# RatInABox-Lab/RatInABox

Measured on AMD Instinct MI355X. Metric: agent-steps/sec (whole node) at 4096 agents x 1024 PlaceCells, higher is better.
Workload: dtype f32 rates / f64 motion

## Files before the change

ratinabox_amd/csrc/riab_handover.h:

```cpp
#pragma once
#include "riab_device.h"

namespace riab {

typedef __attribute__((address_space(1))) uint32_t riab_g32;
typedef __attribute__((address_space(1))) unsigned long long riab_g64;

__device__ __forceinline__ void st_agent(uint32_t* p, uint32_t v) {
  __hip_atomic_store((riab_g32*)(uintptr_t)p, v, __ATOMIC_RELAXED, __HIP_MEMORY_SCOPE_AGENT);
}
__device__ __forceinline__ uint32_t ld_agent(const uint32_t* p) {
  return __hip_atomic_load((riab_g32*)(uintptr_t)p, __ATOMIC_RELAXED, __HIP_MEMORY_SCOPE_AGENT);
}
__device__ __forceinline__ void st_agent(int32_t* p, int32_t v) { st_agent(reinterpret_cast<uint32_t*>(p), (uint32_t)v); }
__device__ __forceinline__ int32_t ld_agent(const int32_t* p) { return (int32_t)ld_agent(reinterpret_cast<const uint32_t*>(p)); }
__device__ __forceinline__ void st_agent(uint64_t* p, uint64_t v) {
  __hip_atomic_store((riab_g64*)(uintptr_t)p, (unsigned long long)v, __ATOMIC_RELAXED, __HIP_MEMORY_SCOPE_AGENT);
}
__device__ __forceinline__ uint64_t ld_agent(const uint64_t* p) {
  return (uint64_t)__hip_atomic_load((riab_g64*)(uintptr_t)p, __ATOMIC_RELAXED, __HIP_MEMORY_SCOPE_AGENT);
}
__device__ __forceinline__ void st_agent(double* p, double v) { st_agent(reinterpret_cast<uint64_t*>(p), (uint64_t)__double_as_longlong(v)); }
__device__ __forceinline__ double ld_agent(const double* p) {
  return __longlong_as_double((long long)ld_agent(reinterpret_cast<const uint64_t*>(p)));
}
__device__ __forceinline__ void st_agent(float* p, float v) { st_agent(reinterpret_cast<uint32_t*>(p), __float_as_uint(v)); }
__device__ __forceinline__ void st_agent(uint8_t* p, uint8_t v) {
  __hip_atomic_store((__attribute__((address_space(1))) uint8_t*)(uintptr_t)p, v, __ATOMIC_RELAXED, __HIP_MEMORY_SCOPE_AGENT);
}
__device__ __forceinline__ uint32_t fetch_add_agent(uint32_t* p, uint32_t v) {
  return __hip_atomic_fetch_add((riab_g32*)(uintptr_t)p, v, __ATOMIC_RELAXED, __HIP_MEMORY_SCOPE_AGENT);
}
__device__ __forceinline__ int32_t fetch_add_agent(int32_t* p, int32_t v) {
  return (int32_t)fetch_add_agent(reinterpret_cast<uint32_t*>(p), (uint32_t)v);
}
__device__ __forceinline__ uint64_t fetch_max_agent(uint64_t* p, uint64_t v) {
  return (uint64_t)__hip_atomic_fetch_max((riab_g64*)(uintptr_t)p, (unsigned long long)v, __ATOMIC_RELAXED, __HIP_MEMORY_SCOPE_AGENT);
}

__device__ __forceinline__ void st_agent_v4f(void* p, riab_v4f v) {
  riab_g64* const g = (riab_g64*)(uintptr_t)p;
  __hip_atomic_store(g, ((unsigned long long)__float_as_uint(v.y) << 32) | __float_as_uint(v.x), __ATOMIC_RELAXED, __HIP_MEMORY_SCOPE_AGENT);
  __hip_atomic_store(g + 1, ((unsigned long long)__float_as_uint(v.w) << 32) | __float_as_uint(v.z), __ATOMIC_RELAXED, __HIP_MEMORY_SCOPE_AGENT);
}
__device__ __forceinline__ riab_v4f ld_agent_v4f(const void* p) {
  riab_g64* const g = (riab_g64*)(uintptr_t)p;
  const unsigned long long lo = __hip_atomic_load(g, __ATOMIC_RELAXED, __HIP_MEMORY_SCOPE_AGENT);
  const unsigned long long hi = __hip_atomic_load(g + 1, __ATOMIC_RELAXED, __HIP_MEMORY_SCOPE_AGENT);
  return riab_v4f{__uint_as_float((uint32_t)lo), __uint_as_float((uint32_t)(lo >> 32)), __uint_as_float((uint32_t)hi),
                  __uint_as_float((uint32_t)(hi >> 32))};
}

__device__ __forceinline__ void drain_stores() { asm volatile("s_waitcnt vmcnt(0)" ::: "memory"); }
#define RIAB_WAITCNT_VMCNT0 0x0F70
__device__ __forceinline__ void drain_stores_nofence_asm() {
  __atomic_signal_fence(__ATOMIC_SEQ_CST);
  __builtin_amdgcn_s_waitcnt(RIAB_WAITCNT_VMCNT0);
  __atomic_signal_fence(__ATOMIC_SEQ_CST);
}

__device__ __forceinline__ uint64_t mail_word(uint32_t epoch, uint32_t v) { return ((uint64_t)epoch << 32) | v; }
__device__ __forceinline__ bool mail_fresh(uint64_t e, uint32_t epoch) { return (uint32_t)(e >> 32) == epoch; }

}
```

ratinabox_amd/csrc/riab_rate_cells.h:

```cpp
#pragma once
#include "riab_device.h"
#include "riab_handover.h"

namespace riab {

typedef float v4f __attribute__((ext_vector_type(4)));
typedef float v2f __attribute__((ext_vector_type(2)));

struct SpikeCtx {
  uint8_t* spikes;
  const float* u_in;
  float dt;
  uint32_t k0, k1;
  uint32_t tag;
};

struct RateArgs {
  const float* pos_x;
  const float* pos_y;
  const float* hd_x;
  const float* hd_y;
  int64_t pos_ld;
  int64_t nquads;
  int64_t qrow;
  int64_t B;
  float* rates;
  uint8_t* spikes;
  const float* u_in;
  float dt, fr_scale, fr_min;
  uint32_t k0, k1;
  uint32_t step0;
  uint32_t tag;
  uint32_t group0;
  int32_t n;
  int32_t cells_per_block;
  __device__ __forceinline__ SpikeCtx spike_ctx() const { return SpikeCtx{spikes, u_in, dt, k0, k1, tag}; }
};

struct PosQuad {
  v4f x, y;
};

__device__ __forceinline__ v4f ldv4(const float* p) { return *reinterpret_cast<const v4f*>(p); }

__device__ __forceinline__ v4f finish_rate(v4f r, const PosQuad& P) {
  r.x = (P.x.x == P.x.x) ? r.x : 0.0f;
  r.y = (P.x.y == P.x.y) ? r.y : 0.0f;
  r.z = (P.x.z == P.x.z) ? r.z : 0.0f;
  r.w = (P.x.w == P.x.w) ? r.w : 0.0f;
  return r;
}
template <class P_>
__device__ __forceinline__ v4f finish_rate(v4f r, const P_&) { return r; }

template <class Cell>
__device__ __forceinline__ v4f post_scale(const Cell&, const float*, const typename Cell::Pos&, v4f r) { return r; }

template <bool EXPLICIT_U, int POLICY = RIAB_STORE_NT>
__device__ __forceinline__ void spike_store(const SpikeCtx& a, v4f r, int64_t off, uint32_t step, uint32_t c,
                                            uint32_t group) {
  v4f u;
  if (EXPLICIT_U) {
    u = ldv4(a.u_in + off);
  } else {
    const u32x4 w = philox4x32_spikes(step, c, group, a.tag, a.k0, a.k1);
    u = v4f{u01_24(w.x), u01_24(w.y), u01_24(w.z), u01_24(w.w)};
  }
  const uint32_t s = (u.x < a.dt * r.x ? 1u : 0u) | (u.y < a.dt * r.y ? 0x100u : 0u) |
                     (u.z < a.dt * r.z ? 0x10000u : 0u) | (u.w < a.dt * r.w ? 0x1000000u : 0u);
  store_stream<POLICY>(reinterpret_cast<uint32_t*>(a.spikes + off), s);
}

template <int DESC, int GX>
struct PlaceCell {
  typedef PosQuad Pos;
  static constexpr int LDS_DOUBLES = (GX == 1 || GX == 2) ? 4 * RIAB_MAX_WALLS + 8 : 1;
  const float* tab;
  float scale, half_scale;
  float top_hat_w2;
  const double* walls;
  int n_internal;
  double e0, e1, e2, e3;
  EnvShape shape;
  const double* lds;

  __device__ __forceinline__ void stage(double* s) {
    lds = s;
    if (GX == 1 || GX == 2) {
      for (int i = threadIdx.x; i < 4 * n_internal; i += 256) s[i] = walls[16 + i];
      __syncthreads();
    }
  }
  __device__ __forceinline__ Pos load(const RateArgs& a, int64_t off) const {
    return Pos{ldv4(a.pos_x + off), ldv4(a.pos_y + off)};
  }
  __device__ __forceinline__ Pos load_agent(const RateArgs& a, int64_t off) const {
    return Pos{ld_agent_v4f(a.pos_x + off), ld_agent_v4f(a.pos_y + off)};
  }
  __device__ __forceinline__ Pos from_rows(v4f x, v4f y, v4f, v4f) const { return Pos{x, y}; }
  static constexpr bool NEEDS_HD = false;
  static constexpr bool NEEDS_POS = true;
  __device__ __forceinline__ float wrap(float v) const {
    const float av = fabsf(v);
    return (av > half_scale) ? -copysignf(scale - av, v) : v;
  }
  __device__ __forceinline__ float dist2(float cxs, float cys, float px, float py) const {
    float dx = cxs - px, dy = cys - py;
    if (GX == 3) {
      dx = wrap(dx);
      dy = wrap(dy);
    }
    float d2 = fmaf(dy, dy, dx * dx);
    if (GX == 1) {
      bool blocked = false;
      for (int w = 0; w < n_internal; ++w)
        blocked |= seg_hit(cxs, cys, px, py, lds[4 * w], lds[4 * w + 1], lds[4 * w + 2], lds[4 * w + 3]);
      if (blocked) d2 = 1.0e6f;
    }
    if (GX == 2) {
      if (n_internal > 0 && seg_hit(cxs, cys, px, py, lds[0], lds[1], lds[2], lds[3])) {
        float best = INFINITY;
        bool any = false;
#pragma unroll
        for (int e = 0; e < 2; ++e) {
          const double exd = lds[2 * e], eyd = lds[2 * e + 1];
          if (env_contains(shape, exd, eyd, [&](int k, double& ax, double& ay, double& bx, double& by) {
                ax = walls[4 * k]; ay = walls[4 * k + 1]; bx = walls[4 * k + 2]; by = walls[4 * k + 3];
              })) {
            const float ex = (float)exd, ey = (float)eyd;
            const float d1 = sqrtf(fmaf(cys - ey, cys - ey, (cxs - ex) * (cxs - ex)));
            const float d2e = sqrtf(fmaf(ey - py, ey - py, (ex - px) * (ex - px)));
            best = fminf(best, d1 + d2e);
            any = true;
          }
        }
        if (any) d2 = best * best;
      }
    }
    return d2;
  }
  __device__ __forceinline__ float fr(float d2, float ks) const {
    if (DESC == RIAB_PC_GAUSSIAN) return __builtin_amdgcn_exp2f(d2 * ks);
    if (DESC == RIAB_PC_GAUSSIAN_THRESHOLD) {
      const float e12 = 0.60653065971263342f;
      return fmaxf(__builtin_amdgcn_exp2f(d2 * ks) - e12, 0.0f) * (1.0f / (1.0f - e12));
    }
    if (DESC == RIAB_PC_DIFF_OF_GAUSSIANS) {
      const float g1 = __builtin_amdgcn_exp2f(d2 * ks);
      const float g2 = __builtin_amdgcn_exp2f(d2 * ks * (1.0f / 2.25f));
      return (g1 - (1.0f / 2.25f) * g2) * (2.25f / 1.25f);
    }
    if (DESC == RIAB_PC_TOP_HAT) return (d2 < top_hat_w2) ? 1.0f : 0.0f;
    return 0.0f;
  }
  static constexpr int NP = 3;
  static constexpr int CPB = 4;
  __device__ __forceinline__ v4f eval(const float* p, const Pos& P) const {
    const float cxs = p[0], cys = p[1], ks = p[2];
    v4f r;
    r.x = fr(dist2(cxs, cys, P.x.x, P.y.x), ks);
    r.y = fr(dist2(cxs, cys, P.x.y, P.y.y), ks);
    r.z = fr(dist2(cxs, cys, P.x.z, P.y.z), ks);
    r.w = fr(dist2(cxs, cys, P.x.w, P.y.w), ks);
    return r;
  }
  template <int D2>
  __host__ PlaceCell<D2, GX> as() const;
};
template <int DESC, int GX>
__host__ __device__ __forceinline__ PlaceCell<DESC, GX> place_cell(const float* tab, float scale, float half_scale, float top_hat_w2,
                                                                   const double* walls = nullptr, int n_internal = 0,
                                                                   const EnvShape& shape = EnvShape{}) {
  PlaceCell<DESC, GX> c;
  c.tab = tab; c.scale = scale; c.half_scale = half_scale; c.top_hat_w2 = top_hat_w2;
  c.walls = walls; c.n_internal = n_internal;
  c.e0 = shape.e0; c.e1 = shape.e1; c.e2 = shape.e2; c.e3 = shape.e3; c.shape = shape; c.lds = nullptr;
  return c;
}
template <int DESC, int GX>
template <int D2>
__host__ PlaceCell<D2, GX> PlaceCell<DESC, GX>::as() const {
  return place_cell<D2, GX>(tab, scale, half_scale, top_hat_w2, walls, n_internal, shape);
}

struct ThetaPos {
  PosQuad q;
  v4f dx, dy;
};

template <int DESC, int GX>
struct ThetaPlaceCell {
  typedef ThetaPos Pos;
  static constexpr int LDS_DOUBLES = 1;
  __device__ __forceinline__ void stage(double*) {}
  PlaceCell<DESC, GX> base;
  const float* tab;
  const double* vx64;
  const double* vy64;
  float phase0;
  float k2;
  float norm;
  __device__ __forceinline__ Pos load(const RateArgs& a, int64_t off) const {
    Pos P;
    P.q = base.load(a, off);
    const double* px = vx64 + off;
    const double* py = vy64 + off;
    const v4f vx = {(float)px[0], (float)px[1], (float)px[2], (float)px[3]};
    const v4f vy = {(float)py[0], (float)py[1], (float)py[2], (float)py[3]};
    const v4f sp{sqrtf(fmaf(vy.x, vy.x, vx.x * vx.x)), sqrtf(fmaf(vy.y, vy.y, vx.y * vx.y)),
                 sqrtf(fmaf(vy.z, vy.z, vx.z * vx.z)), sqrtf(fmaf(vy.w, vy.w, vx.w * vx.w))};
    const v4f inv = 1.0f / (sp + 1e-8f);
    P.dx = vx * inv;
    P.dy = vy * inv;
    return P;
  }
  static constexpr int NP = 4;
  static constexpr int CPB = 4;
  __device__ __forceinline__ v4f eval(const float* p, const Pos& P) const { return base.eval(p, P.q); }
  __device__ __forceinline__ float factor(float cx, float cy, float pf, float px, float py, float dx, float dy) const {
    const float along = fmaf(py - cy, dy, (px - cx) * dx);
    float rev = fmaf(-along, pf, phase0);
    rev -= floorf(rev);
    return __builtin_amdgcn_exp2f((__builtin_amdgcn_cosf(rev) - 1.0f) * k2) * norm;
  }
  __device__ __forceinline__ v4f modulation(const float* p, const Pos& P) const {
    return v4f{factor(p[0], p[1], p[3], P.q.x.x, P.q.y.x, P.dx.x, P.dy.x), factor(p[0], p[1], p[3], P.q.x.y, P.q.y.y, P.dx.y, P.dy.y),
               factor(p[0], p[1], p[3], P.q.x.z, P.q.y.z, P.dx.z, P.dy.z), factor(p[0], p[1], p[3], P.q.x.w, P.q.y.w, P.dx.w, P.dy.w)};
  }
};

template <int DESC, int GX>
__device__ __forceinline__ v4f post_scale(const ThetaPlaceCell<DESC, GX>& c, const float* p, const ThetaPos& P, v4f r) {
  return r * c.modulation(p, P);
}
__device__ __forceinline__ v4f finish_rate(v4f r, const ThetaPos& P) { return finish_rate(r, P.q); }

template <int DESC>
struct GridCell {
  typedef PosQuad Pos;
  static constexpr int LDS_DOUBLES = 1;
  __device__ __forceinline__ void stage(double*) {}
  const float* tab;
  float f0, inv_1mf0;
  __device__ __forceinline__ Pos load(const RateArgs& a, int64_t off) const {
    return Pos{ldv4(a.pos_x + off), ldv4(a.pos_y + off)};
  }
  __device__ __forceinline__ Pos load_agent(const RateArgs& a, int64_t off) const {
    return Pos{ld_agent_v4f(a.pos_x + off), ld_agent_v4f(a.pos_y + off)};
  }
  __device__ __forceinline__ Pos from_rows(v4f x, v4f y, v4f, v4f) const { return Pos{x, y}; }
  static constexpr bool NEEDS_HD = false;
  static constexpr bool NEEDS_POS = true;
  __device__ __forceinline__ v2f two(const float* p, v2f x, v2f y) const {
    v2f s = {0.0f, 0.0f};
#pragma unroll
    for (int i = 0; i < 3; ++i) {
      const v2f p0 = {p[3 * i], p[3 * i]}, p1 = {p[3 * i + 1], p[3 * i + 1]}, p2 = {p[3 * i + 2], p[3 * i + 2]};
      v2f rev = p0 - __builtin_elementwise_fma(x, p1, y * p2);
      rev.x -= floorf(rev.x);
      rev.y -= floorf(rev.y);
      s += v2f{__builtin_amdgcn_cosf(rev.x), __builtin_amdgcn_cosf(rev.y)};
    }
    s *= v2f{1.0f / 3.0f, 1.0f / 3.0f};
    if (DESC == RIAB_GC_RECTIFIED) {
      const v2f r = (s - v2f{f0, f0}) * v2f{inv_1mf0, inv_1mf0};
      return v2f{fmaxf(r.x, 0.0f), fmaxf(r.y, 0.0f)};
    }
    return v2f{2.0f / 3.0f, 2.0f / 3.0f} * (s + v2f{0.5f, 0.5f});
  }
  static constexpr int NP = 9;
  static constexpr int CPB = 4;
  __device__ __forceinline__ v4f eval(const float* p, const Pos& P) const {
    const v2f lo = two(p, v2f{P.x.x, P.x.y}, v2f{P.y.x, P.y.y});
    const v2f hi = two(p, v2f{P.x.z, P.x.w}, v2f{P.y.z, P.y.w});
    return v4f{lo.x, lo.y, hi.x, hi.y};
  }
};

struct PlaneWaveCell {
  typedef PosQuad Pos;
  static constexpr int LDS_DOUBLES = 1;
  __device__ __forceinline__ void stage(double*) {}
  const float* tab;
  __device__ __forceinline__ Pos load(const RateArgs& a, int64_t off) const {
    return Pos{ldv4(a.pos_x + off), ldv4(a.pos_y + off)};
  }
  __device__ __forceinline__ Pos load_agent(const RateArgs& a, int64_t off) const {
    return Pos{ld_agent_v4f(a.pos_x + off), ld_agent_v4f(a.pos_y + off)};
  }
  __device__ __forceinline__ Pos from_rows(v4f x, v4f y, v4f, v4f) const { return Pos{x, y}; }
  static constexpr bool NEEDS_HD = false;
  static constexpr bool NEEDS_POS = true;
  __device__ __forceinline__ v2f two(const float* p, v2f x, v2f y) const {
#pragma clang fp contract(off)
    const v2f p0 = {p[0], p[0]}, p1 = {p[1], p[1]}, p2 = {p[2], p[2]};
    v2f rev = p0 - __builtin_elementwise_fma(x, p1, y * p2);
    rev.x -= floorf(rev.x);
    rev.y -= floorf(rev.y);
    const v2f c = {__builtin_amdgcn_cosf(rev.x), __builtin_amdgcn_cosf(rev.y)};
    return __builtin_elementwise_fma(v2f{0.5f, 0.5f}, c, v2f{0.5f, 0.5f});
  }
  static constexpr int NP = 3;
  static constexpr int CPB = 4;
  __device__ __forceinline__ v4f eval(const float* p, const Pos& P) const {
    const v2f lo = two(p, v2f{P.x.x, P.x.y}, v2f{P.y.x, P.y.y});
    const v2f hi = two(p, v2f{P.x.z, P.x.w}, v2f{P.y.z, P.y.w});
    return v4f{lo.x, lo.y, hi.x, hi.y};
  }
};

template <int MODE>
struct HDCell {
  struct Pos {
    v4f cs, sn;
    v4f speed;
  };
  static constexpr int LDS_DOUBLES = 1;
  __device__ __forceinline__ void stage(double*) {}
  const float* tab;
  float speed_inv;
  const double* vx64;
  const double* vy64;
  __device__ __forceinline__ Pos load_agent(const RateArgs& a, int64_t off) const {
    return from_dirs(ld_agent_v4f(a.hd_x + off), ld_agent_v4f(a.hd_y + off));
  }
  __device__ __forceinline__ Pos from_rows(v4f, v4f, v4f hx, v4f hy) const { return from_dirs(hx, hy); }
  static constexpr bool NEEDS_HD = true;
  static constexpr bool NEEDS_POS = false;
  __device__ __forceinline__ Pos load(const RateArgs& a, int64_t off) const {
    v4f hx, hy;
    if (MODE == 1 && vx64) {
      const double* px = vx64 + off;
      const double* py = vy64 + off;
      hx = v4f{(float)px[0], (float)px[1], (float)px[2], (float)px[3]};
      hy = v4f{(float)py[0], (float)py[1], (float)py[2], (float)py[3]};
    } else {
      hx = ldv4(a.hd_x + off);
      hy = ldv4(a.hd_y + off);
    }
    return from_dirs(hx, hy);
  }
  __device__ __forceinline__ Pos from_dirs(v4f hx, v4f hy) const {
    Pos P;
    if (MODE >= 1) {
      const v4f sp{sqrtf(fmaf(hy.x, hy.x, hx.x * hx.x)), sqrtf(fmaf(hy.y, hy.y, hx.y * hx.y)),
                   sqrtf(fmaf(hy.z, hy.z, hx.z * hx.z)), sqrtf(fmaf(hy.w, hy.w, hx.w * hx.w))};
      P.speed = sp * speed_inv;
      if (MODE == 1) {
        hx = hx / sp;
        hy = hy / sp;
      }
    } else {
      P.speed = v4f{1.0f, 1.0f, 1.0f, 1.0f};
    }
    {
#pragma clang fp contract(off)
      const v4f bx = hx + 1e-6f;
      const v4f inv = {1.0f / sqrtf(fmaf(hy.x, hy.x, bx.x * bx.x)), 1.0f / sqrtf(fmaf(hy.y, hy.y, bx.y * bx.y)),
                       1.0f / sqrtf(fmaf(hy.z, hy.z, bx.z * bx.z)), 1.0f / sqrtf(fmaf(hy.w, hy.w, bx.w * bx.w))};
      P.cs = bx * inv;
      P.sn = hy * inv;
    }
    return P;
  }
  static constexpr int NP = 3;
  static constexpr int CPB = 16;
  __device__ __forceinline__ v4f eval(const float* p, const Pos& P) const {
#pragma clang fp contract(off)
    if (MODE == 2) return P.speed;
    const float cp = p[0], sp = p[1], k2 = p[2];
    const v4f cosd = __builtin_elementwise_fma(P.cs, v4f{cp, cp, cp, cp}, P.sn * sp);
    const v4f dc = P.cs - cp, ds = P.sn - sp;
    const v4f chord = __builtin_elementwise_fma(ds, ds, dc * dc) * -0.5f;
    const v4f prod = cosd - 1.0f;
    const v4f e = v4f{cosd.x > 0.75f ? chord.x : prod.x, cosd.y > 0.75f ? chord.y : prod.y, cosd.z > 0.75f ? chord.z : prod.z,
                      cosd.w > 0.75f ? chord.w : prod.w} * k2;
    return v4f{__builtin_amdgcn_exp2f(e.x), __builtin_amdgcn_exp2f(e.y), __builtin_amdgcn_exp2f(e.z),
               __builtin_amdgcn_exp2f(e.w)};
  }
};

__device__ __forceinline__ v4f finish_rate(v4f r, const HDCell<1>::Pos& P) { return r * P.speed; }

#define RIAB_CELL_GROUP(Cell, CPB, cell, mine, P, c0, n, fr_scale, fr_min, rates, off, ld, store, RATE_POLICY, PHILOX,       \
                        EXPLICIT, SPIKE_POLICY, ctx, step, group)                                                         \
  {                                                                                                                        \
    static_assert(Cell::NP * (CPB) <= 64, "a cell group's parameters must fit one wave");                                  \
    _Pragma("unroll") for (int j_ = 0; j_ < (CPB); ++j_) {                                                                 \
      if ((c0) + j_ < (n)) {                                                                             \
        float p_[Cell::NP];                                                                                                \
        _Pragma("unroll") for (int i_ = 0; i_ < Cell::NP; ++i_) p_[i_] = __builtin_bit_cast(                               \
            float, __builtin_amdgcn_readlane(__builtin_bit_cast(int, mine), j_ * Cell::NP + i_));                          \
        v4f r_ = (cell).eval(p_, P);                                                                                       \
        r_ = finish_rate(post_scale(cell, p_, P, r_ * (fr_scale) + (fr_min)), P);           \
        if (store) {                                                                                                       \
          store_stream<(RATE_POLICY)>((rates) + (off), r_);                                                                \
          if (PHILOX) spike_store<false, (SPIKE_POLICY)>(ctx, r_, off, step, (uint32_t)((c0) + j_), group);                \
          if (EXPLICIT) spike_store<true, (SPIKE_POLICY)>(ctx, r_, off, step, (uint32_t)((c0) + j_), group);               \
        }                                                                                                                  \
        (off) += (ld);                                                                                                     \
      }                                                                                                                    \
    }                                                                                                                      \
  }

}
```

ratinabox_amd/csrc/riab_rates.hip:

```cpp
#include <hip/hip_ext.h>

#include <type_traits>

#include "riab_device.h"
#include "riab_rate_cells.h"
#include "riab_handover.h"
#include "riab_launch.h"
#ifndef RIAB_SPIKE_POLICY_GATED
#define RIAB_SPIKE_POLICY_GATED RIAB_STORE_NT
#endif
#ifndef RIAB_SPIKE_POLICY_WIDE
#define RIAB_SPIKE_POLICY_WIDE RIAB_STORE_NT
#endif

namespace riab {


template <class Cell, int SPK, int CPB, bool NT>
__global__ __launch_bounds__(256) void rate_kernel_wide(const RateArgs a, Cell cell) {
  __shared__ double s_lds[Cell::LDS_DOUBLES];
  cell.stage(s_lds);
  constexpr int NP = Cell::NP;
  const int lane = threadIdx.x & 63;
  const int c0 = blockIdx.y * CPB;
  const uint32_t t = blockIdx.z;
  const uint32_t q = blockIdx.x * 256u + threadIdx.x;
  const bool live = q < (uint32_t)a.qrow;
  const uint32_t qc = live ? q : 0u;
  const int pi = c0 * NP + lane;
  const float mine = (lane < NP * CPB && pi < a.n * NP) ? cell.tab[pi] : 0.0f;
  const typename Cell::Pos P = cell.load(a, (int64_t)t * a.pos_ld + 4 * (int64_t)qc);
  int64_t off = ((int64_t)t * a.n + c0) * a.B + 4 * (int64_t)qc;
  const uint32_t step = a.step0 + t;
  const uint32_t group = a.group0 + qc;
  const SpikeCtx k = a.spike_ctx();
  RIAB_CELL_GROUP(Cell, CPB, cell, mine, P, c0, a.n, a.fr_scale, a.fr_min, a.rates, off, a.B, live,
                  NT ? RIAB_STORE_WT : RIAB_STORE_PLAIN, SPK == 1, SPK == 2, NT ? RIAB_STORE_WT : RIAB_SPIKE_POLICY_WIDE, k, step, group)
}

template <class Cell, int SPK>
__global__ __launch_bounds__(256) void rate_kernel_generic(const RateArgs a, Cell cell) {
  __shared__ double s_lds[Cell::LDS_DOUBLES];
  cell.stage(s_lds);
  constexpr int NP = Cell::NP;
  const uint32_t p4 = blockIdx.x * 256u + threadIdx.x;
  const bool live = p4 < a.nquads;
  const uint32_t pc = live ? p4 : 0u;
  const uint32_t t = pc / (uint32_t)a.qrow;
  const uint32_t q = pc - t * (uint32_t)a.qrow;
  const typename Cell::Pos P = cell.load(a, (int64_t)t * a.pos_ld + 4 * (int64_t)q);
  const int c0 = blockIdx.y * a.cells_per_block;
  const int c1 = min(a.n, c0 + a.cells_per_block);
  int64_t off = ((int64_t)t * a.n + c0) * a.B + 4 * (int64_t)q;
  const uint32_t step = a.step0 + t;
  const uint32_t group = a.group0 + q;
  const int lane = threadIdx.x & 63;
  for (int cb = c0; cb < c1; cb += 64) {
    float mine[NP];
    const int cm = min(cb + lane, a.n - 1);
#pragma unroll
    for (int i = 0; i < NP; ++i) mine[i] = cell.tab[cm * NP + i];
    const int cnt = min(64, c1 - cb);
    for (int j = 0; j < cnt; ++j) {
      float p[NP];
#pragma unroll
      for (int i = 0; i < NP; ++i)
        p[i] = __builtin_bit_cast(float, __builtin_amdgcn_readlane(__builtin_bit_cast(int, mine[i]), j));
      v4f r = cell.eval(p, P);
      r = finish_rate(post_scale(cell, p, P, r * a.fr_scale + a.fr_min), P);
      if (live) {
        store_stream<RIAB_STORE_NT>(a.rates + off, r);
        if (SPK == 1) spike_store<false>(a.spike_ctx(), r, off, step, (uint32_t)(cb + j), group);
        if (SPK == 2) spike_store<true>(a.spike_ctx(), r, off, step, (uint32_t)(cb + j), group);
      }
      off += a.B;
    }
  }
}

template <int GX>
__global__ __launch_bounds__(256) void place_one_hot_kernel(const RateArgs a, PlaceCell<RIAB_PC_GAUSSIAN, GX> cell) {
  __shared__ double s_lds[PlaceCell<RIAB_PC_GAUSSIAN, GX>::LDS_DOUBLES];
  cell.stage(s_lds);
  const uint32_t p4 = blockIdx.x * 256u + threadIdx.x;
// ... 92 lines not shown
    off += a.B;
  }
}

__global__ __launch_bounds__(256) void noise_kernel(float* noise, float* rates, const float* z_in, int n,
                                                    int64_t qrow, int T, float theta_dt, float sigma_dt, uint32_t k0,
                                                    uint32_t k1, uint32_t step0, uint32_t tag, uint32_t group0) {
  const int64_t q = (int64_t)blockIdx.x * 256 + threadIdx.x;
  if (q >= qrow) return;
  const int64_t row = (int64_t)n * qrow * 4;
  for (int c = blockIdx.y; c < n; c += gridDim.y) {
    const int64_t off = ((int64_t)c * qrow + q) * 4;
    v4f x = ldv4(noise + off);
    for (int t = 0; t < T; ++t) {
      v4f z;
      if (z_in) {
        z = ldv4(z_in + t * row + off);
      } else {
        const u32x4 w = philox4x32_spikes(step0 + (uint32_t)t, (uint32_t)c, group0 + (uint32_t)q, tag, k0, k1);
        const float u0 = ((float)(w.x >> 8) + 0.5f) * 0x1.0p-24f, u1 = (float)(w.y >> 8) * 0x1.0p-24f;
        const float u2 = ((float)(w.z >> 8) + 0.5f) * 0x1.0p-24f, u3 = (float)(w.w >> 8) * 0x1.0p-24f;
        const float r0 = sqrtf(-2.0f * logf(u0)), r1 = sqrtf(-2.0f * logf(u2));
        z = v4f{r0 * __builtin_amdgcn_cosf(u1), r0 * __builtin_amdgcn_sinf(u1), r1 * __builtin_amdgcn_cosf(u3),
                r1 * __builtin_amdgcn_sinf(u3)};
      }
      x = x + (-theta_dt) * x + sigma_dt * z;
      const v4f r = ldv4(rates + t * row + off);
      *reinterpret_cast<v4f*>(rates + t * row + off) = r + x;
    }
    *reinterpret_cast<v4f*>(noise + off) = x;
  }
}

__global__ __launch_bounds__(256) void fill_kernel(float* dst, int64_t n4, float value) {
  const int64_t i = (int64_t)blockIdx.x * 256 + threadIdx.x;
  if (i < n4) reinterpret_cast<v4f*>(dst)[i] = v4f{value, value, value, value};
}

struct StreamArgs {
  uint32_t* ctrl;
  uint32_t step_base;
  uint32_t spin_limit;
  uint32_t stamps;
  uint32_t sleep_max;
  uint32_t serial_rows;
  uint32_t serial_gap;
};
__device__ __forceinline__ bool ended_just_now(const uint32_t* ctrl, uint32_t gap_ticks) {
  const unsigned long long end = ld_agent(reinterpret_cast<const uint64_t*>(ctrl + RIAB_CTRL_TRAJ_STAMPS + 2));
  const unsigned long long now = __builtin_amdgcn_s_memrealtime();
  return now >= end && now - end < (unsigned long long)gap_ticks;
}
__device__ __forceinline__ int stream_progress(const StreamArgs& s, uint32_t q, int lane) {
  int rel = 0x7fffffff;
  if (lane < 4) {
    const uint32_t v = ld_agent(s.ctrl + RIAB_CTRL_PROGRESS + 32 * q + lane);
    rel = (int)(v - s.step_base);
    rel = rel < 0 ? 0 : rel;
  }
  const int r0 = __builtin_amdgcn_readlane(rel, 0), r1 = __builtin_amdgcn_readlane(rel, 1);
  const int r2 = __builtin_amdgcn_readlane(rel, 2), r3 = __builtin_amdgcn_readlane(rel, 3);
  return __builtin_amdgcn_readfirstlane(min(min(r0, r1), min(r2, r3)));
}
__device__ __forceinline__ void stream_wait(const StreamArgs& s, uint32_t q, int t, int lane) {
  int known = stream_progress(s, q, lane);
  for (uint32_t spins = 0; known <= t; ++spins) {
    const uint32_t ab = ld_agent(s.ctrl + RIAB_CTRL_ABORT);
    if (__builtin_amdgcn_readfirstlane((int)ab)) return;
    if (spins >= s.spin_limit) {
      if (lane == 0) {
        atomicAdd(s.ctrl + RIAB_CTRL_TIMEOUTS, 1u);
        st_agent(s.ctrl + RIAB_CTRL_ABORT, 1u);
      }
      return;
    }
    if (spins < 4) __builtin_amdgcn_s_sleep(4);
    else if (spins < 16 || s.sleep_max <= 16) __builtin_amdgcn_s_sleep(16);
    else if (s.sleep_max >= 48) __builtin_amdgcn_s_sleep(48);
    else __builtin_amdgcn_s_sleep(32);
    known = stream_progress(s, q, lane);
  }
}

template <class Cell, int SPK, int CPB, bool LONG, int WAVES>
__global__ __launch_bounds__(64 * WAVES) void rate_kernel_gated(const RateArgs a, Cell cell, const StreamArgs s) {
  __shared__ double s_lds[Cell::LDS_DOUBLES];
  cell.stage(s_lds);
  constexpr int NP = Cell::NP;
  static_assert(WAVES % 4 == 0, "four waves share a (1024 agents) x (CPB cells) tile");
  const int lane = threadIdx.x & 63;
  const int wv = __builtin_amdgcn_readfirstlane((int)(threadIdx.x >> 6));
  const int c0 = (int)(blockIdx.y * (WAVES / 4) + (wv >> 2)) * CPB;
  const uint32_t t = blockIdx.z;
  const uint32_t q = blockIdx.x * 256u + (threadIdx.x & 255u);
  const uint32_t wq = (uint32_t)__builtin_amdgcn_readfirstlane((int)(blockIdx.x * 4u + (uint32_t)(wv & 3)));
  if (wq * 64u >= (uint32_t)a.qrow || c0 >= a.n) return;
  const int pi = c0 * NP + lane;
  const float mine = (lane < NP * CPB && pi < a.n * NP) ? cell.tab[pi] : 0.0f;
  const bool grid_first = t == 0 && blockIdx.x == 0 && blockIdx.y == 0 && wv == 0;
  if (s.stamps && grid_first && lane == 0)
    st_agent(reinterpret_cast<uint64_t*>(s.ctrl + RIAB_CTRL_STAMPS), (uint64_t)__builtin_amdgcn_s_memrealtime());
  if (s.serial_rows >= 8u && grid_first) {
    if (stream_progress(s, wq, lane) >= (int)s.serial_rows && ended_just_now(s.ctrl, s.serial_gap) && lane == 0)
      atomicAdd(s.ctrl + RIAB_CTRL_SERIALISED, 1u);
  }
#ifdef RIAB_PIPE_PROFILE
  riab_g64* const dbg = (riab_g64*)(uintptr_t)(s.ctrl + 2048);
  const bool first_wg = blockIdx.x == 0 && blockIdx.y == 0 && threadIdx.x == 0;
  if (first_wg) dbg[1 * 64 + t] = (unsigned long long)__builtin_amdgcn_s_memrealtime();
#endif
  stream_wait(s, wq, (int)t, lane);
#ifdef RIAB_PIPE_PROFILE
  if (first_wg) dbg[2 * 64 + t] = (unsigned long long)__builtin_amdgcn_s_memrealtime();
#endif
  const int64_t po = (int64_t)t * a.pos_ld + 4 * (int64_t)q;
  const typename Cell::Pos P = cell.load_agent(a, po);
  int64_t off = ((int64_t)t * a.n + c0) * a.B + 4 * (int64_t)q;
  const uint32_t step = a.step0 + t;
  const uint32_t group = a.group0 + q;
  const SpikeCtx k = a.spike_ctx();
  RIAB_CELL_GROUP(Cell, CPB, cell, mine, P, c0, a.n, a.fr_scale, a.fr_min, a.rates, off, a.B, true, RIAB_STORE_NT, SPK == 1, false,
                  RIAB_SPIKE_POLICY_GATED, k, step, group)
#ifdef RIAB_PIPE_PROFILE
  if (c0 + CPB >= a.n && blockIdx.x + 1 == gridDim.x && (threadIdx.x & 255u) == 0) {
    drain_stores();
    dbg[3 * 64 + t] = (unsigned long long)__builtin_amdgcn_s_memrealtime();
  }
#endif
  if (s.stamps && t + 1 == gridDim.z && c0 + CPB >= a.n) {
    drain_stores();
    if (lane == 0) fetch_max_agent(reinterpret_cast<uint64_t*>(s.ctrl + RIAB_CTRL_STAMPS + 2), (uint64_t)__builtin_amdgcn_s_memrealtime());
  }
}

__global__ __launch_bounds__(64) void stream_gate_kernel(uint32_t* ctrl, uint32_t started_target, uint32_t n_traj,
                                                         uint32_t progress_target, uint32_t spin_limit, uint32_t sleep_long,
                                                         uint32_t final_target, uint32_t serial_gap) {
  const int lane = threadIdx.x;
  for (uint32_t spins = 0;; ++spins) {
    const uint32_t v = ld_agent(ctrl + RIAB_CTRL_STARTED);
    bool ok = (int32_t)(v - started_target) >= 0;
    bool all_done = ok && final_target != 0u && spins == 0u;
    if (ok) {
      for (uint32_t w = lane; w < n_traj; w += 64) {
        const uint32_t p = ld_agent(ctrl + RIAB_CTRL_PROGRESS_WORD(w));
        ok = ok && (int32_t)(p - progress_target) >= 0;
        all_done = all_done && (int32_t)(p - final_target) >= 0;
      }
    }
    if (spins == 0u && final_target != 0u && n_traj > 0u && __builtin_amdgcn_ballot_w64(!all_done) == 0 &&
        ended_just_now(ctrl, serial_gap) && lane == 0)
      atomicAdd(ctrl + RIAB_CTRL_SERIALISED, 1u);
    if (__builtin_amdgcn_ballot_w64(!ok) == 0) return;
    if (ld_agent(ctrl + RIAB_CTRL_ABORT)) return;
    if (spins >= spin_limit) {
      if (lane == 0) {
        atomicAdd(ctrl + RIAB_CTRL_TIMEOUTS, 1u);
        st_agent(ctrl + RIAB_CTRL_ABORT, 1u);
      }
      return;
    }
    if (sleep_long && spins >= 64) __builtin_amdgcn_s_sleep(127);
    else if (sleep_long) __builtin_amdgcn_s_sleep(8);
    else __builtin_amdgcn_s_sleep(16);
  }
}

__global__ __launch_bounds__(64) void stream_open_kernel(uint32_t* ctrl, uint32_t n_traj, uint32_t step_base) {
  for (uint32_t w = threadIdx.x; w < n_traj; w += 64)
    st_agent(ctrl + RIAB_CTRL_PROGRESS_WORD(w), step_base);
  if (threadIdx.x == 0)
    st_agent(ctrl + RIAB_CTRL_STARTED, 0u);
}

static int check_io(const RiabRateIO* io, int n, bool need_pos, bool need_hd) {
  if (!io || n <= 0 || io->T <= 0 || io->B <= 0 || !io->rates) return RIAB_EINVAL;
  if (need_pos && (!io->pos_x || !io->pos_y)) return RIAB_EINVAL;
  if (need_hd && (!io->hd_x || !io->hd_y)) return RIAB_EINVAL;
  if (io->B % 4 != 0 || io->pos_ld % 4 != 0 || io->agent_id0 % 4 != 0) return RIAB_EALIGN;
  const uintptr_t m = (uintptr_t)io->rates | (uintptr_t)io->pos_x | (uintptr_t)io->pos_y | (uintptr_t)io->hd_x |
                      (uintptr_t)io->hd_y | (uintptr_t)io->u_in;
  if (m & 15) return RIAB_EALIGN;
  if ((uintptr_t)io->spikes & 3) return RIAB_EALIGN;
  if (io->u_in && !io->spikes) return RIAB_EINVAL;
  if (io->T * (io->B / 4) >= ((int64_t)1 << 31)) return RIAB_ETOOBIG;
  return RIAB_OK;
}

static RateArgs make_args(const RiabRateIO* io, int n) {
  RateArgs a;
  a.pos_x = io->pos_x;
  a.pos_y = io->pos_y;
  a.hd_x = io->hd_x;
  a.hd_y = io->hd_y;
  a.pos_ld = io->pos_ld;
  a.qrow = io->B / 4;
  a.nquads = io->T * a.qrow;
  a.B = io->B;
  a.rates = io->rates;
  a.spikes = io->spikes;
  a.u_in = io->u_in;
  a.dt = io->dt;
  a.fr_scale = io->max_fr - io->min_fr;
  a.fr_min = io->min_fr;
  a.k0 = (uint32_t)io->seed;
// ... 40 lines not shown

static int place_geometry_refused(const RiabEnv* env, int geometry) {
  if (env->periodic) return geometry != RIAB_GEOM_EUCLIDEAN ? RIAB_EUNSUPPORTED : RIAB_OK;
  if (geometry == RIAB_GEOM_EUCLIDEAN) return RIAB_OK;
  if (env->n_walls - 4 > RIAB_MAX_WALLS) return RIAB_ETOOBIG;
  if (geometry == RIAB_GEOM_GEODESIC && env->n_walls > 5) return RIAB_EUNSUPPORTED;
  return RIAB_OK;
}
static int place_geometry_check(const RiabEnv* env, int geometry) {
  if (!env->periodic && geometry != RIAB_GEOM_EUCLIDEAN && env->n_walls > 4 && !env->walls) return RIAB_EINVAL;
  return place_geometry_refused(env, geometry);
}
template <class F>
static int visit_place_geometry(const RiabEnv* env, int geometry, F&& f) {
  if (env->periodic) return f(std::integral_constant<int, 3>{});
  switch (geometry) {
    case RIAB_GEOM_EUCLIDEAN: return f(std::integral_constant<int, 0>{});
    case RIAB_GEOM_LINE_OF_SIGHT: return f(std::integral_constant<int, 1>{});
    case RIAB_GEOM_GEODESIC: return f(std::integral_constant<int, 2>{});
    default: return RIAB_EINVAL;
  }
}
template <int GX>
static int internal_walls(const RiabEnv* env) {
  const int n_internal = env->n_walls > 4 ? env->n_walls - 4 : 0;
  return (GX == 2 && n_internal > 1) ? 1 : n_internal;
}
template <int GX>
static PlaceCell<RIAB_PC_GAUSSIAN, GX> make_place_cell(const RiabEnv* env, const float* table, float top_hat_width, int n_internal) {
  return place_cell<RIAB_PC_GAUSSIAN, GX>(table, (float)env->scale, (float)(env->scale / 2), top_hat_width * top_hat_width,
                                          env->walls, n_internal, make_env_shape(env));
}
template <int GX, class F>
static int visit_place_desc(int desc, const PlaceCell<RIAB_PC_GAUSSIAN, GX>& base, int otherwise, F&& f) {
  switch (desc) {
    case RIAB_PC_GAUSSIAN: return f(base);
    case RIAB_PC_GAUSSIAN_THRESHOLD: return f(base.template as<RIAB_PC_GAUSSIAN_THRESHOLD>());
    case RIAB_PC_DIFF_OF_GAUSSIANS: return f(base.template as<RIAB_PC_DIFF_OF_GAUSSIANS>());
    case RIAB_PC_TOP_HAT: return f(base.template as<RIAB_PC_TOP_HAT>());
    default: return otherwise;
  }
}
template <class F>
static int visit_grid_desc(int desc, const float* table, float f0, F&& f) {
  if (desc == RIAB_GC_RECTIFIED) return f(GridCell<RIAB_GC_RECTIFIED>{table, f0, 1.0f / (1.0f - f0)});
  if (desc == RIAB_GC_SHIFTED) return f(GridCell<RIAB_GC_SHIFTED>{table, f0, 1.0f});
  return RIAB_EINVAL;
}

template <int GX>
static int launch_place(const RiabRateIO* io, int n, int desc, const PlaceCell<RIAB_PC_GAUSSIAN, GX>& base,
                        hipStream_t s) {
  if (desc == RIAB_PC_ONE_HOT) {
    RateArgs a = make_args(io, n);
    dim3 grid = generic_grid(&a);
    grid.y = 1;
    hipLaunchKernelGGL((place_one_hot_kernel<GX>), grid, dim3(256), 0, s, a, base);
    return (int)hipGetLastError();
  }
  return visit_place_desc(desc, base, RIAB_EINVAL, [&](const auto& c) { return launch_rate(io, n, c, s); });
}

static uint32_t serial_gap_ticks() {
  static uint32_t ticks = 0;
  if (!ticks) {
    int dev = 0, khz = 0;
    if (hipGetDevice(&dev) != hipSuccess || hipDeviceGetAttribute(&khz, hipDeviceAttributeWallClockRate, dev) != hipSuccess || khz <= 0)
      khz = 100000;
    ticks = (uint32_t)((long long)khz * 25 / 1000);
  }
  return ticks;
}

struct StreamLaunch {
  StreamArgs st;
  hipEvent_t ev0, ev1;
  int T;
  bool spikes;
  bool reserve;
  bool dry_run;
  hipStream_t s;
};

template <class Cell>
static int launch_stream_cell(const RateArgs& a, const Cell& cell, const StreamLaunch& L) {
  constexpr int CPB = (Cell::NP * 2 * Cell::CPB <= 64) ? 2 * Cell::CPB : Cell::CPB;
  using Kernel = void (*)(const RateArgs, Cell, const StreamArgs);
  static constexpr Kernel kGated[8] = {
      rate_kernel_gated<Cell, 0, CPB, false, 4>,  rate_kernel_gated<Cell, 0, CPB, true, 4>,
      rate_kernel_gated<Cell, 1, CPB, false, 4>,  rate_kernel_gated<Cell, 1, CPB, true, 4>,
      rate_kernel_gated<Cell, 0, CPB, false, 12>, rate_kernel_gated<Cell, 0, CPB, true, 12>,
      rate_kernel_gated<Cell, 1, CPB, false, 12>, rate_kernel_gated<Cell, 1, CPB, true, 12>};
  const int T = L.T;
  const int64_t groups = (a.n + CPB - 1) / CPB;
  if (T > 65535 || groups > 65535) return RIAB_ETOOBIG;
  const bool reserve = L.reserve;
  const int variant = (reserve ? 4 : 0) + (L.spikes ? 2 : 0) + (T > 256 ? 1 : 0);
  if (reserve) {
    static int regs[8] = {0, 0, 0, 0, 0, 0, 0, 0};
    int& r = regs[variant];
    if (r == 0) {
      hipFuncAttributes attr;
      const void* f = (const void*)kGated[variant];
      r = (hipFuncGetAttributes(&attr, f) == hipSuccess && attr.numRegs > 0) ? attr.numRegs : 1 << 20;
      if (r < (1 << 20) && 2 * (int64_t)attr.sharedSizeBytes + 81920 > 160 * 1024) r = 1 << 20;
      (void)hipGetLastError();
    }
    if (6 * ((r + 7) / 8 * 8) + traj_kernel_regs() > 512) return RIAB_EUNSUPPORTED;
  }
  if (L.dry_run) return RIAB_OK;
  static bool launched[8] = {false, false, false, false, false, false, false, false};
  bool& seen = launched[variant];
  StreamArgs st = L.st;
  if (!seen) st.serial_rows = 0u;
  seen = true;
  const dim3 grid((unsigned)((a.qrow + 255) / 256), (unsigned)(reserve ? (groups + 2) / 3 : groups), (unsigned)T);
  const dim3 block(reserve ? 768 : 256);
  if (L.ev0 || L.ev1) hipExtLaunchKernelGGL(kGated[variant], grid, block, 0, L.s, L.ev0, L.ev1, 0u, a, cell, st);
  else hipLaunchKernelGGL(kGated[variant], grid, block, 0, L.s, a, cell, st);
  return (int)hipGetLastError();
}

template <class F>
static int visit_stream_cell(const RiabEnv* env, const RiabPopulation* pop, F&& f) {
  switch (pop->kind) {
    case RIAB_POP_PLACE:
      return visit_place_geometry(env, pop->geometry, [&](auto gx) {
        return visit_place_desc(pop->description, make_place_cell<decltype(gx)::value>(env, pop->table, pop->top_hat_width, internal_walls<decltype(gx)::value>(env)),
                                RIAB_EUNSUPPORTED, f);
      });
    case RIAB_POP_GRID: return visit_grid_desc(pop->description, pop->table, pop->f0, f);
    case RIAB_POP_HDC: return f(HDCell<0>{pop->table, 0.0f, nullptr, nullptr});
    case RIAB_POP_PLANE_WAVE: return f(PlaneWaveCell{pop->table});
    default: return RIAB_EUNSUPPORTED;
  }
}

int stream_supported(const RiabEnv* env, const RiabPopulation* pop, int64_t B) {
  if (!env || !pop || pop->n <= 0 || B <= 0 || B % 256 != 0) return RIAB_EUNSUPPORTED;
  if (pop->noise_state) return RIAB_EUNSUPPORTED;
  switch (pop->kind) {
    case RIAB_POP_PLACE:
      if (pop->description == RIAB_PC_ONE_HOT) return RIAB_EUNSUPPORTED;
      if (place_geometry_refused(env, pop->geometry)) return RIAB_EUNSUPPORTED;
      return pop->table ? RIAB_OK : RIAB_EINVAL;
    case RIAB_POP_GRID:
    case RIAB_POP_HDC:
    case RIAB_POP_PLANE_WAVE: return pop->table ? RIAB_OK : RIAB_EINVAL;
    default: return RIAB_EUNSUPPORTED;
  }
}

int launch_rate_stream(const RiabEnv* env, const RiabPopulation* pop, const float* hist, int64_t B, int32_t T, float dt,
                       uint64_t seed, uint64_t step0, int64_t agent_id0, uint32_t* ctrl, uint32_t spin_limit, bool stamps,
                       hipStream_t s, hipEvent_t ev_start, hipEvent_t ev_stop, bool dry_run, bool reserve,
                       uint32_t serial_rows) {
  int rc = stream_supported(env, pop, B);
  if (rc) return rc;
  if (!hist || !ctrl || !pop->rates_base || T <= 0 || pop->capacity_rows < T || agent_id0 % 4) return RIAB_EINVAL;
  if ((((uintptr_t)hist | (uintptr_t)pop->rates_base) & 15) || ((uintptr_t)pop->spikes_base & 3)) return RIAB_EALIGN;
  RiabRateIO io = pop->io;
  hist_rows_io(&io, hist, B, (int64_t)RIAB_HIST_ROWS * B);
  io.T = T;
  io.rates = pop->rates_base;
  io.spikes = pop->spikes_base;
  io.u_in = nullptr;
  io.dt = dt;
  io.seed = seed;
  io.step0 = step0 + 1;
  io.agent_id0 = agent_id0;
  const RateArgs a = make_args(&io, pop->n);
  StreamArgs st;
  st.ctrl = ctrl;
  st.step_base = (uint32_t)step0;
  st.spin_limit = spin_limit;
  st.stamps = stamps ? 1u : 0u;
  st.sleep_max = (uint32_t)g_options[RIAB_OPT_POLL_SLEEP];
  st.serial_rows = serial_rows;
  st.serial_gap = serial_gap_ticks();
  const StreamLaunch L{st, ev_start, ev_stop, T, pop->spikes_base != nullptr, reserve, dry_run, s};
  return visit_stream_cell(env, pop, [&](const auto& c) { return launch_stream_cell(a, c, L); });
}

int launch_stream_open(uint32_t* ctrl, uint32_t n_traj, uint32_t step_base, hipStream_t s) {
  hipLaunchKernelGGL(stream_open_kernel, dim3(1), dim3(64), 0, s, ctrl, n_traj, step_base);
  return (int)hipGetLastError();
}

int launch_stream_gate(uint32_t* ctrl, uint32_t started_target, uint32_t n_traj, uint32_t progress_target,
                       uint32_t spin_limit, bool sleep_long, uint32_t final_target, hipStream_t s) {
  static bool launched = false;
  if (!launched) final_target = 0u;
  launched = true;
  hipLaunchKernelGGL(stream_gate_kernel, dim3(1), dim3(64), 0, s, ctrl, started_target, n_traj, progress_target, spin_limit,
                     sleep_long ? 1u : 0u, final_target, serial_gap_ticks());
  return (int)hipGetLastError();
}

}

using namespace riab;

// ... 202 lines not shown
```

Measured before the change: 1.421 billion.

## Add per-wave cell-run rate kernel with LDS-shared positions and paired agent loads

Adds a RUNS variant of the gated streaming rate kernel. Each wave of a 256-thread block now owns a contiguous slice of CPB/4 cells instead of all four waves sharing the same cells. The block stages its 1024 agent positions in LDS so every wave evaluates all four quads and writes contiguous rows for its cells. Agent-scope position and head-direction loads are also replaced by one inline-asm pair of dwordx4 loads with a single waitcnt. The variant is picked by default for long, non-spiking, non-reserved runs with B divisible by 1024, can be turned off with an env var, and adds a __syncthreads plus LDS traffic.

```diff
diff --git a/ratinabox_amd/csrc/riab_handover.h b/ratinabox_amd/csrc/riab_handover.h
--- a/ratinabox_amd/csrc/riab_handover.h
+++ b/ratinabox_amd/csrc/riab_handover.h
@@ -50,6 +50,10 @@
   return riab_v4f{__uint_as_float((uint32_t)lo), __uint_as_float((uint32_t)(lo >> 32)), __uint_as_float((uint32_t)hi),
                   __uint_as_float((uint32_t)(hi >> 32))};
 }
+__device__ __forceinline__ void ld_agent_v4f_pair(const void* px, const void* py, riab_v4f& x, riab_v4f& y) {
+  asm volatile("global_load_dwordx4 %0, %2, off sc1\n\tglobal_load_dwordx4 %1, %3, off sc1\n\ts_waitcnt vmcnt(0)"
+               : "=&v"(x), "=&v"(y) : "v"(px), "v"(py) : "memory");
+}
 
 __device__ __forceinline__ void drain_stores() { asm volatile("s_waitcnt vmcnt(0)" ::: "memory"); }
 #define RIAB_WAITCNT_VMCNT0 0x0F70
diff --git a/ratinabox_amd/csrc/riab_rate_cells.h b/ratinabox_amd/csrc/riab_rate_cells.h
--- a/ratinabox_amd/csrc/riab_rate_cells.h
+++ b/ratinabox_amd/csrc/riab_rate_cells.h
@@ -95,7 +95,9 @@
     return Pos{ldv4(a.pos_x + off), ldv4(a.pos_y + off)};
   }
   __device__ __forceinline__ Pos load_agent(const RateArgs& a, int64_t off) const {
-    return Pos{ld_agent_v4f(a.pos_x + off), ld_agent_v4f(a.pos_y + off)};
+    Pos P;
+    ld_agent_v4f_pair(a.pos_x + off, a.pos_y + off, P.x, P.y);
+    return P;
   }
   __device__ __forceinline__ Pos from_rows(v4f x, v4f y, v4f, v4f) const { return Pos{x, y}; }
   static constexpr bool NEEDS_HD = false;
@@ -246,7 +248,9 @@
     return Pos{ldv4(a.pos_x + off), ldv4(a.pos_y + off)};
   }
   __device__ __forceinline__ Pos load_agent(const RateArgs& a, int64_t off) const {
-    return Pos{ld_agent_v4f(a.pos_x + off), ld_agent_v4f(a.pos_y + off)};
+    Pos P;
+    ld_agent_v4f_pair(a.pos_x + off, a.pos_y + off, P.x, P.y);
+    return P;
   }
   __device__ __forceinline__ Pos from_rows(v4f x, v4f y, v4f, v4f) const { return Pos{x, y}; }
   static constexpr bool NEEDS_HD = false;
@@ -286,7 +290,9 @@
     return Pos{ldv4(a.pos_x + off), ldv4(a.pos_y + off)};
   }
   __device__ __forceinline__ Pos load_agent(const RateArgs& a, int64_t off) const {
-    return Pos{ld_agent_v4f(a.pos_x + off), ld_agent_v4f(a.pos_y + off)};
+    Pos P;
+    ld_agent_v4f_pair(a.pos_x + off, a.pos_y + off, P.x, P.y);
+    return P;
   }
   __device__ __forceinline__ Pos from_rows(v4f x, v4f y, v4f, v4f) const { return Pos{x, y}; }
   static constexpr bool NEEDS_HD = false;
@@ -322,7 +328,9 @@
   const double* vx64;
   const double* vy64;
   __device__ __forceinline__ Pos load_agent(const RateArgs& a, int64_t off) const {
-    return from_dirs(ld_agent_v4f(a.hd_x + off), ld_agent_v4f(a.hd_y + off));
+    v4f hx, hy;
+    ld_agent_v4f_pair(a.hd_x + off, a.hd_y + off, hx, hy);
+    return from_dirs(hx, hy);
   }
   __device__ __forceinline__ Pos from_rows(v4f, v4f, v4f hx, v4f hy) const { return from_dirs(hx, hy); }
   static constexpr bool NEEDS_HD = true;
@@ -403,4 +411,22 @@
     }                                                                                                                      \
   }
 
-}
+#define RIAB_CELL_RUNS(Cell, CPW, cell, mine, PV, c0, n, fr_scale, fr_min, rates, off, ld, RATE_POLICY)                     \
+  {                                                                                                                        \
+    static_assert(Cell::NP * (CPW) <= 64, "a wave's cells' parameters must fit one wave");                                 \
+    _Pragma("unroll") for (int j_ = 0; j_ < (CPW); ++j_) {                                                                 \
+      if ((c0) + j_ < (n)) {                                                                             \
+        float p_[Cell::NP];                                                                                                \
+        _Pragma("unroll") for (int i_ = 0; i_ < Cell::NP; ++i_) p_[i_] = __builtin_bit_cast(                               \
+            float, __builtin_amdgcn_readlane(__builtin_bit_cast(int, mine), j_ * Cell::NP + i_));                          \
+        _Pragma("unroll") for (int k_ = 0; k_ < 4; ++k_) {                                                                 \
+          v4f r_ = (cell).eval(p_, (PV)[k_]);                                                                              \
+          r_ = finish_rate(post_scale(cell, p_, (PV)[k_], r_ * (fr_scale) + (fr_min)), (PV)[k_]);                          \
+          store_stream<(RATE_POLICY)>((rates) + (off) + 256 * k_, r_);                                                     \
+        }                                                                                                                  \
+        (off) += (ld);                                                                                                     \
+      }                                                                                                                    \
+    }                                                                                                                      \
+  }
+
+}
diff --git a/ratinabox_amd/csrc/riab_rates.hip b/ratinabox_amd/csrc/riab_rates.hip
--- a/ratinabox_amd/csrc/riab_rates.hip
+++ b/ratinabox_amd/csrc/riab_rates.hip
@@ -1,5 +1,7 @@
 #include <hip/hip_ext.h>
 
+#include <cstdlib>
+#include <cstring>
 #include <type_traits>
 
 #include "riab_device.h"
@@ -258,21 +260,26 @@
   }
 }
 
-template <class Cell, int SPK, int CPB, bool LONG, int WAVES>
+template <class Cell, int SPK, int CPB, bool LONG, int WAVES, bool RUNS = false>
 __global__ __launch_bounds__(64 * WAVES) void rate_kernel_gated(const RateArgs a, Cell cell, const StreamArgs s) {
   __shared__ double s_lds[Cell::LDS_DOUBLES];
+  __shared__ v4f s_pos[RUNS ? 2 : 1][RUNS ? 256 : 1];
   cell.stage(s_lds);
   constexpr int NP = Cell::NP;
   static_assert(WAVES % 4 == 0, "four waves share a (1024 agents) x (CPB cells) tile");
+  static_assert(!RUNS || (LONG && WAVES == 4 && SPK == 0 && CPB % 4 == 0 && Cell::LDS_DOUBLES == 1 &&
+                          sizeof(typename Cell::Pos) == 2 * sizeof(v4f)), "the RUNS shape: see above");
+  constexpr int CPW = CPB / 4;
   const int lane = threadIdx.x & 63;
   const int wv = __builtin_amdgcn_readfirstlane((int)(threadIdx.x >> 6));
   const int c0 = (int)(blockIdx.y * (WAVES / 4) + (wv >> 2)) * CPB;
   const uint32_t t = blockIdx.z;
   const uint32_t q = blockIdx.x * 256u + (threadIdx.x & 255u);
   const uint32_t wq = (uint32_t)__builtin_amdgcn_readfirstlane((int)(blockIdx.x * 4u + (uint32_t)(wv & 3)));
-  if (wq * 64u >= (uint32_t)a.qrow || c0 >= a.n) return;
-  const int pi = c0 * NP + lane;
-  const float mine = (lane < NP * CPB && pi < a.n * NP) ? cell.tab[pi] : 0.0f;
+  if ((!RUNS && wq * 64u >= (uint32_t)a.qrow) || c0 >= a.n) return;
+  const int cw = RUNS ? c0 + CPW * wv : c0;
+  const int pi = cw * NP + lane;
+  const float mine = (lane < NP * (RUNS ? CPW : CPB) && pi < a.n * NP) ? cell.tab[pi] : 0.0f;
   const bool grid_first = t == 0 && blockIdx.x == 0 && blockIdx.y == 0 && wv == 0;
   if (s.stamps && grid_first && lane == 0)
     st_agent(reinterpret_cast<uint64_t*>(s.ctrl + RIAB_CTRL_STAMPS), (uint64_t)__builtin_amdgcn_s_memrealtime());
@@ -295,8 +302,19 @@
   const uint32_t step = a.step0 + t;
   const uint32_t group = a.group0 + q;
   const SpikeCtx k = a.spike_ctx();
-  RIAB_CELL_GROUP(Cell, CPB, cell, mine, P, c0, a.n, a.fr_scale, a.fr_min, a.rates, off, a.B, true, RIAB_STORE_NT, SPK == 1, false,
-                  RIAB_SPIKE_POLICY_GATED, k, step, group)
+  if constexpr (RUNS) {
+    s_pos[0][threadIdx.x] = P.x;
+    s_pos[1][threadIdx.x] = P.y;
+    __syncthreads();
+    typename Cell::Pos PV[4];
+#pragma unroll
+    for (int k_ = 0; k_ < 4; ++k_) PV[k_] = typename Cell::Pos{s_pos[0][64 * k_ + lane], s_pos[1][64 * k_ + lane]};
+    int64_t offw = ((int64_t)t * a.n + cw) * a.B + 1024 * (int64_t)blockIdx.x + 4 * lane;
+    RIAB_CELL_RUNS(Cell, CPW, cell, mine, PV, cw, a.n, a.fr_scale, a.fr_min, a.rates, offw, a.B, RIAB_STORE_NT)
+  } else {
+    RIAB_CELL_GROUP(Cell, CPB, cell, mine, P, c0, a.n, a.fr_scale, a.fr_min, a.rates, off, a.B, true, RIAB_STORE_NT, SPK == 1, false,
+                    RIAB_SPIKE_POLICY_GATED, k, step, group)
+  }
 #ifdef RIAB_PIPE_PROFILE
   if (c0 + CPB >= a.n && blockIdx.x + 1 == gridDim.x && (threadIdx.x & 255u) == 0) {
     drain_stores();
@@ -503,6 +521,21 @@
   hipStream_t s;
 };
 
+static bool stream_shape_rows() {
+  static const bool rows = [] {
+    const char* v = getenv("RIAB_STREAM_SHAPE");
+    return v && !strcmp(v, "rows");
+  }();
+  return rows;
+}
+
+template <class Cell, int CPB>
+static auto stream_runs_kernel() -> void (*)(const RateArgs, Cell, const StreamArgs) {
+  if constexpr (Cell::LDS_DOUBLES == 1 && sizeof(typename Cell::Pos) == 2 * sizeof(v4f) && CPB % 4 == 0)
+    return rate_kernel_gated<Cell, 0, CPB, true, 4, true>;
+  else return nullptr;
+}
+
 template <class Cell>
 static int launch_stream_cell(const RateArgs& a, const Cell& cell, const StreamLaunch& L) {
   constexpr int CPB = (Cell::NP * 2 * Cell::CPB <= 64) ? 2 * Cell::CPB : Cell::CPB;
@@ -529,16 +562,32 @@
     }
     if (6 * ((r + 7) / 8 * 8) + traj_kernel_regs() > 512) return RIAB_EUNSUPPORTED;
   }
+  Kernel kernel = kGated[variant];
+  bool runs = false;
+  if (T > 256 && !reserve && !L.spikes && a.B % 1024 == 0 && !stream_shape_rows()) {
+    if (const Kernel kr = stream_runs_kernel<Cell, CPB>()) {
+      static int fits = -1;
+      if (fits < 0) {
+        hipFuncAttributes attr;
+        fits = (hipFuncGetAttributes(&attr, (const void*)kr) == hipSuccess && 8 * (int64_t)attr.sharedSizeBytes + 81920 <= 160 * 1024) ? 1 : 0;
+        (void)hipGetLastError();
+      }
+      if (fits) {
+        kernel = kr;
+        runs = true;
+      }
+    }
+  }
   if (L.dry_run) return RIAB_OK;
-  static bool launched[8] = {false, false, false, false, false, false, false, false};
-  bool& seen = launched[variant];
+  static bool launched[9] = {false, false, false, false, false, false, false, false, false};
+  bool& seen = launched[runs ? 8 : variant];
   StreamArgs st = L.st;
   if (!seen) st.serial_rows = 0u;
   seen = true;
   const dim3 grid((unsigned)((a.qrow + 255) / 256), (unsigned)(reserve ? (groups + 2) / 3 : groups), (unsigned)T);
   const dim3 block(reserve ? 768 : 256);
-  if (L.ev0 || L.ev1) hipExtLaunchKernelGGL(kGated[variant], grid, block, 0, L.s, L.ev0, L.ev1, 0u, a, cell, st);
-  else hipLaunchKernelGGL(kGated[variant], grid, block, 0, L.s, a, cell, st);
+  if (L.ev0 || L.ev1) hipExtLaunchKernelGGL(kernel, grid, block, 0, L.s, L.ev0, L.ev1, 0u, a, cell, st);
+  else hipLaunchKernelGGL(kernel, grid, block, 0, L.s, a, cell, st);
   return (int)hipGetLastError();
 }
 
```

New measurement: 1.301 billion. 0.916x the previous value.
